# Tencent/hpc-ops

Measured on AMD Instinct MI355X. Metric: attention_decode_fp8_kv_throughput, higher is better.
Workload: dtype fp8_e4m3

## Files before the change

hpc-ops_amd/csrc/attention_decode_v2.hip:

```cpp
#include <atomic>
#include <type_traits>
#include <utility>

#include "hpc_common.h"
#include "hpc_dev.h"
#include "../../include/hpc_amd.h"
#include "attention_decode_v2.h"

namespace hpc {
namespace decode2 {

#ifdef HPC_DEV
__device__ int g_ticket_overruns;
#endif
constexpr int kThreads = 256;
constexpr int kWaves = 4;
constexpr float kNegInf = -__builtin_inff();
constexpr int kRow = 256;
constexpr int kRows = 32;
constexpr int kVOff = kRows * kRow;
constexpr int kWaveLds = 2 * kRows * kRow;

template <int kAux>
__device__ __forceinline__ void ld_x4x4(u32x4 (&k)[4], int voff, i32x4 rs_in, int s1, int s2, int s3) {
  const i32x4 rs = pin(rs_in);
  if constexpr (kAux == 2)
    asm volatile("s_nop 4\n\tbuffer_load_dwordx4 %0, %4, %5, 0 offen nt\n\tbuffer_load_dwordx4 %1, %4, %5, %6 offen nt\n\t"
                 "buffer_load_dwordx4 %2, %4, %5, %7 offen nt\n\tbuffer_load_dwordx4 %3, %4, %5, %8 offen nt"
                 : "=&v"(k[0]), "=&v"(k[1]), "=&v"(k[2]), "=&v"(k[3])
                 : "v"(voff), "s"(rs), "s"(s1), "s"(s2), "s"(s3));
  else
    asm volatile("s_nop 4\n\tbuffer_load_dwordx4 %0, %4, %5, 0 offen\n\tbuffer_load_dwordx4 %1, %4, %5, %6 offen\n\t"
                 "buffer_load_dwordx4 %2, %4, %5, %7 offen\n\tbuffer_load_dwordx4 %3, %4, %5, %8 offen"
                 : "=&v"(k[0]), "=&v"(k[1]), "=&v"(k[2]), "=&v"(k[3])
                 : "v"(voff), "s"(rs), "s"(s1), "s"(s2), "s"(s3));
}
__device__ __forceinline__ void ld_q3(u32x4 (&q)[2], uint32_t& sc, int voff_q, i32x4 rq_in, int voff_s, i32x4 rsc_in) {
  const i32x4 rq = pin(rq_in), rsc = pin(rsc_in);
  asm volatile("s_nop 4\n\tbuffer_load_dwordx4 %0, %3, %4, 0 offen\n\tbuffer_load_dwordx4 %1, %3, %4, 0 offen offset:64\n\t"
               "buffer_load_dword %2, %5, %6, 0 offen"
               : "=&v"(q[0]), "=&v"(q[1]), "=&v"(sc)
               : "v"(voff_q), "s"(rq), "v"(voff_s), "s"(rsc));
}
__device__ __forceinline__ void ld_q4(u32x4 (&q)[4], int voff_q, i32x4 rq_in) {
  const i32x4 rq = pin(rq_in);
  asm volatile("s_nop 4\n\tbuffer_load_dwordx4 %0, %4, %5, 0 offen\n\tbuffer_load_dwordx4 %1, %4, %5, 0 offen offset:64\n\t"
               "buffer_load_dwordx4 %2, %4, %5, 0 offen offset:128\n\tbuffer_load_dwordx4 %3, %4, %5, 0 offen offset:192"
               : "=&v"(q[0]), "=&v"(q[1]), "=&v"(q[2]), "=&v"(q[3])
               : "v"(voff_q), "s"(rq));
}
__device__ __forceinline__ void ld_ks(uint32_t& sc, int voff, i32x4 rs_in) {
  const i32x4 rs = pin(rs_in);
  asm volatile("s_nop 4\n\tbuffer_load_dword %0, %1, %2, 0 offen" : "=&v"(sc) : "v"(voff), "s"(rs));
}
template <int N>
__device__ __forceinline__ void wait_ks(uint32_t& sc) {
  asm volatile("s_waitcnt vmcnt(%1)" : "+v"(sc) : "n"(N));
}
template <int N>
__device__ __forceinline__ void wait_ks2(uint32_t& sc0, uint32_t& sc1) {
  asm volatile("s_waitcnt vmcnt(%2)" : "+v"(sc0), "+v"(sc1) : "n"(N));
}
template <int N>
__device__ __forceinline__ void wait_q8(u32x4 (&q0)[4], u32x4 (&q1)[4]) {
  asm volatile("s_waitcnt vmcnt(%8)"
               : "+v"(q0[0]), "+v"(q0[1]), "+v"(q0[2]), "+v"(q0[3]), "+v"(q1[0]), "+v"(q1[1]), "+v"(q1[2]), "+v"(q1[3])
               : "n"(N < 63 ? N : 63));
}
template <int N>
__device__ __forceinline__ void wait_x4x4(u32x4 (&k)[4]) {
  asm volatile("s_waitcnt vmcnt(%4)" : "+v"(k[0]), "+v"(k[1]), "+v"(k[2]), "+v"(k[3]) : "n"(N < 63 ? N : 63));
}
template <int N>
__device__ __forceinline__ void wait_q(u32x4 (&q0)[2], u32x4 (&q1)[2], uint32_t& s0, uint32_t& s1) {
  asm volatile("s_waitcnt vmcnt(%6)" : "+v"(q0[0]), "+v"(q0[1]), "+v"(q1[0]), "+v"(q1[1]), "+v"(s0), "+v"(s1) : "n"(N < 63 ? N : 63));
}


constexpr int kFValid = 1;
constexpr int kFLast = 2;
constexpr int kFFirst = 4;
constexpr int kFOn0 = 8;
constexpr int kFOn1 = 16;
constexpr int kFMasked = 32;

template <int kAux, bool kBf16 = false, bool kProf = false, bool kQuad = false, bool kKtok = false, bool kHnd = false, bool kSolo = false>
__global__ __launch_bounds__(kThreads, 2) void decode2_kernel(const Args a) {
  static_assert(!kSolo || (!kQuad && !kHnd), "one head per workgroup: fp8 (both quant types) or bf16");
  static_assert(!(kSolo && kBf16 && kKtok), "bf16 has no scales");
  static_assert(!(kBf16 && kQuad), "the quad form is fp8");
  static_assert(!kKtok || (!kBf16 && !kQuad), "per-token K scales: the fp8 head-pair form");
  static_assert(!kHnd || (!kBf16 && !kQuad && !kKtok), "HND pages: the fp8 head-pair form with per-tensor scales");
  __shared__ float s_ks[kKtok ? kWaves : 1][64];
  constexpr bool kWide = (kBf16 && !kSolo) || kQuad;
  constexpr bool kBSolo = kBf16 && kSolo;
  __shared__ __attribute__((aligned(1024))) uint8_t s_wave[kWaves][kWaveLds];
  __shared__ float s_m[2][kWaves][16];
  __shared__ float s_l[2][kWaves][16];
  __shared__ int s_ticket[2];
  constexpr int kH = kSolo ? 1 : kQuad ? 4 : 2;
  constexpr int kW = kBSolo ? 32 : kSolo ? 64 : kWide ? 16 : 32;
  constexpr int kRowB = kBSolo ? 256 : kSolo ? 128 : kWide ? 512 : 256;
  constexpr int kRpi = kBSolo ? 4 : (kHnd || kSolo) ? 8 : kWide ? 2 : 4;
  constexpr int kCpr = 64 / kRpi;

  const int tid = threadIdx.x;
  const int lane = tid & 63;
  const int wave = sgpr(tid >> 6);
  const int n = lane & 15;
  const int g = lane >> 4;
  const int wg = blockIdx.x, nwg = gridDim.x;
  const int B = a.num_batch, Sq = a.num_seq_q;
  const int G = 1 << a.g_shift;
  const int rows_valid = Sq << a.g_shift;
  auto row_ok = [&](int r16, int hh = 0) __attribute__((always_inline)) { return (kQuad ? (r16 & 7) : kSolo ? 16 * hh + r16 : r16) < rows_valid; };
  const int page_mask = (1 << a.page_shift) - 1;
  const cint_ptr lens = as_const(a.lens);
  const int mpl_tiles = as_const(a.task_map)[6] >> 6;
  const int add_new = a.new_kv_included ? 0 : Sq;
  const uint8_t* qbase = static_cast<const uint8_t*>(a.q);
  const auto part_rs = make_rsrc(a.part_o);
  const auto lse_rs = make_rsrc(a.part_lse);
  auto ltot_of = [&](int b) __attribute__((always_inline)) { const int l = lens[b] + add_new; return l > 0 ? l : 0; };
  auto tiles_of = [&](int b) __attribute__((always_inline)) { return (ltot_of(b) + 63) >> 6; };

  constexpr int kOvh = 2;
  auto cost_of = [&](int b) __attribute__((always_inline)) { const int t = tiles_of(b); return t > 0 ? t + kOvh : 0; };
  const int kpl = (B + 63) >> 6;
  int chunk_sum = 0;
  for (int i = 0; i < kpl; ++i) {
    const int b = lane * kpl + i;
    if (b < B) {
      const int l = a.lens[b] + add_new;
      const int t = ((l > 0 ? l : 0) + 63) >> 6;
      chunk_sum += t > 0 ? t + kOvh : 0;
    }
  }
  int incl = chunk_sum;
  incl += __builtin_amdgcn_update_dpp(0, incl, 0x111, 0xF, 0xF, false);
  incl += __builtin_amdgcn_update_dpp(0, incl, 0x112, 0xF, 0xF, false);
  incl += __builtin_amdgcn_update_dpp(0, incl, 0x114, 0xF, 0xF, false);
  incl += __builtin_amdgcn_update_dpp(0, incl, 0x118, 0xF, 0xF, false);
  incl += __builtin_amdgcn_update_dpp(0, incl, 0x142, 0xA, 0xF, false);
  incl += __builtin_amdgcn_update_dpp(0, incl, 0x143, 0xC, 0xF, false);
  const int chunk_start = incl - chunk_sum;
  const int Th = __builtin_amdgcn_readlane(incl, 63);
  const int npair = a.num_head_kv / kH;
  if (Th == 0) return;
  int nrange = nwg / npair;
  int rng = wg / npair;
  int pr = wg % npair;
  if (a.xcd_map != 0 && npair == 4 && (nwg & 7) == 0) {
    const int e = (a.xcd_map >> (3 * (wg & 7))) & 7;
    pr = e & 3;
    rng = (wg >> 3) * 2 + (e >> 2);
  }
  if (a.mate_from > 0 && wg >= a.mate_from) pr ^= a.pair_xor;
  if constexpr (kSolo) {
    if (a.share_shift > 0) {
      const int ss = a.share_shift, hk = npair >> ss;
      if (hk < 8 && (8 % hk) == 0 && (nrange % (8 / hk)) == 0) {
        const int x = wg & 7, j = wg >> 3;
        pr = ((x % hk) << ss) | (j & ((1 << ss) - 1));
        rng = (j >> ss) * (8 / hk) + x / hk;
      } else {
        pr = ((pr % hk) << ss) | (pr / hk);
      }
    }
  }
  int lwg = wg;
  int lwg0 = pr * nrange;
  if (a.pair_wgs[0] > 0 && npair == 4) {
    const int n0 = a.pair_wgs[0], n1 = a.pair_wgs[1], n2 = a.pair_wgs[2], n3 = a.pair_wgs[3];
    const int nmin = min(min(n0, n1), min(n2, n3));
    if (wg >= nmin * 4) {
      int e = wg - nmin * 4;
      pr = 0;
      rng = nmin + e;
      if (e >= n0 - nmin) { e -= n0 - nmin; pr = 1; rng = nmin + e;
        if (e >= n1 - nmin) { e -= n1 - nmin; pr = 2; rng = nmin + e;
          if (e >= n2 - nmin) { e -= n2 - nmin; pr = 3; rng = nmin + e; } } }
    }
    nrange = pr == 0 ? n0 : pr == 1 ? n1 : pr == 2 ? n2 : n3;
    lwg0 = pr == 0 ? 0 : pr == 1 ? n0 : pr == 2 ? n0 + n1 : n0 + n1 + n2;
  }
  lwg = lwg0 + rng;
  const int nbig = a.big_pct > 100 ? (nwg / 2) / npair : 0;
  const long denom = static_cast<long>(nbig) * a.big_pct + static_cast<long>(nrange - nbig) * 100;
  const int per_s_even = static_cast<int>((static_cast<long>(Th) * 100 + denom - 1) / denom);
  const int per_floor = a.min_range_cost > mpl_tiles ? a.min_range_cost : mpl_tiles;
  const int per_s = per_s_even > per_floor ? per_s_even : per_floor;
  const int per_b = nbig > 0 ? (per_s * a.big_pct + 99) / 100 : per_s;
  const int big_span = nbig * per_b;
  auto range_of = [&](int pos) __attribute__((always_inline)) { return pos < big_span ? pos / per_b : nbig + (pos - big_span) / per_s; };
  const long g_begin = rng < nbig ? static_cast<long>(rng) * per_b : big_span + static_cast<long>(rng - nbig) * per_s;
  const int per = rng < nbig ? per_b : per_s;
  const long g_end = g_begin + per < Th ? g_begin + per : Th;
  if (g_begin >= g_end) return;

  constexpr int kSnap = 16;
  const bool snap = per_s_even <= per_floor && !(kHpcDevBuild && a.dev_nosnap);
  auto locate = [&](int x, int& b_out, int& rt_out, int& cc_out) __attribute__((always_inline)) {
    if (x >= Th) {
      b_out = B;
      rt_out = 0;
      cc_out = Th;
      return;
    }
    const uint64_t le = __ballot(chunk_start <= x);
    const int cl = 63 - __builtin_clzll(le);
    int pos = __builtin_amdgcn_readlane(chunk_start, cl);
    int b = cl * kpl;
    while (true) {
      const int t = cost_of(b);
      if (x < pos + t) break;
      pos += t;
      ++b;
    }
    if (snap && x > pos) {
      const int t = cost_of(b);
      if (t - kOvh <= kSnap) {
        if (2 * (x - pos) >= t) {
          pos += t;
          ++b;
          while (b < B && cost_of(b) == 0) ++b;
          if (b >= B) {
            b_out = B;
            rt_out = 0;
            cc_out = Th;
            return;
          }
        }
        b_out = b;
        rt_out = 0;
        cc_out = pos;
        return;
      }
    }
    b_out = b;
    rt_out = x - pos > kOvh ? x - pos - kOvh : 0;
    cc_out = pos;
  };
  int c_b, c_rt0, c_cc, e_b, e_rt, e_cc;
  locate(static_cast<int>(g_begin), c_b, c_rt0, c_cc);
  locate(static_cast<int>(g_end), e_b, e_rt, e_cc);
  if (c_b == e_b && c_rt0 >= e_rt) return;

  int q0_b = 0, q0_ltot = 0, q0_end = 0, q0_cc = 0;
  int q1_b = 0, q1_ltot = 0, q1_end = 0, q1_cc = 0;
  int q2_b = 0, q2_ltot = 0, q2_end = 0, q2_cc = 0;
  int qn = 0;
  int c_tok = 0, c_tok_end = 0, c_ltot = 0, c_tiles = 0, c_first = 1, c_valid = 1, c_pending = 0, c_last = 0;
  cint_ptr c_row = as_const(a.block_ids);
  auto open_task = [&]() __attribute__((always_inline)) {
    c_ltot = ltot_of(c_b);
    c_tiles = (c_ltot + 63) >> 6;
    const int end_t = c_b == e_b ? e_rt : c_tiles;
    c_tok_end = end_t * 64 < c_ltot ? end_t * 64 : c_ltot;
    c_tok = c_rt0 * 64 + wave * kW;
    c_first = 1;
    c_row = as_const(a.block_ids) + static_cast<long>(c_b) * a.max_blocks;
    const bool e0 = qn == 0, e1 = qn == 1, e2 = qn >= 2;
    q0_b = e0 ? c_b : q0_b, q0_ltot = e0 ? c_ltot : q0_ltot, q0_end = e0 ? c_tok_end : q0_end, q0_cc = e0 ? c_cc : q0_cc;
    q1_b = e1 ? c_b : q1_b, q1_ltot = e1 ? c_ltot : q1_ltot, q1_end = e1 ? c_tok_end : q1_end, q1_cc = e1 ? c_cc : q1_cc;
    q2_b = e2 ? c_b : q2_b, q2_ltot = e2 ? c_ltot : q2_ltot, q2_end = e2 ? c_tok_end : q2_end, q2_cc = e2 ? c_cc : q2_cc;
    ++qn;
  };
  auto next_task = [&]() __attribute__((always_inline)) {
    if (c_b == e_b) {
      c_valid = 0;
      return;
    }
    c_cc += c_tiles + kOvh;
    do {
      ++c_b;
    } while (c_b < e_b && tiles_of(c_b) == 0);
    if (c_b == e_b && e_rt == 0) {
      c_valid = 0;
      return;
    }
    c_rt0 = 0;
    open_task();
  };
  const bool blk1_same_page = (1 << a.page_shift) >= kW;
  auto step = [&](int& tok, int& fl, int& pid0, int& pid1) __attribute__((always_inline)) {
    if (c_pending && c_valid) {
      if (c_last) {
        next_task();
      } else {
        c_tok += kWaves * kW;
        c_first = 0;
      }
    }
    c_pending = 1;
    c_last = c_tok + kWaves * kW >= c_tok_end;
    const bool on0 = c_valid && c_tok < c_tok_end, on1 = c_valid && c_tok + kW / 2 < c_tok_end;
    const bool masked = c_tok + kW > c_ltot - Sq + 1 || c_tok + kW > c_tok_end;
    fl = (c_valid ? kFValid : 0) | (c_last ? kFLast : 0) | (c_first ? kFFirst : 0) | (on0 ? kFOn0 : 0) | (on1 ? kFOn1 : 0) |
         (masked ? kFMasked : 0);
    tok = c_tok;
    pid0 = on0 ? c_row[c_tok >> a.page_shift] : 0;
    pid1 = (!blk1_same_page && on1) ? c_row[(c_tok + kW / 2) >> a.page_shift] : 0;
  };

  u32x4 kr[2][4];
  u32x4 vr[2][4];
  uint32_t qsc[2];
  const uint32_t k_rs = static_cast<uint32_t>(a.k_token_stride), v_rs = static_cast<uint32_t>(a.v_token_stride);
  const int in0 = (wave * kW) & page_mask;
  const int in1 = blk1_same_page ? in0 + kW / 2 : ((wave * kW + kW / 2) & page_mask);
  const int lane_off = (lane % kCpr) * 16;
  const int k_voff0 = static_cast<int>((in0 + lane / kCpr) * k_rs) + lane_off, k_voff1 = static_cast<int>((in1 + lane / kCpr) * k_rs) + lane_off;
  const int v_voff0 = static_cast<int>((in0 + lane / kCpr) * v_rs) + lane_off, v_voff1 = static_cast<int>((in1 + lane / kCpr) * v_rs) + lane_off;
  const int ks1 = sgpr(kRpi * k_rs), ks2 = sgpr(kHnd ? static_cast<uint32_t>(a.k_head_stride) : 2 * kRpi * k_rs);
  const int ks3 = sgpr(kHnd ? static_cast<uint32_t>(a.k_head_stride) + kRpi * k_rs : 3 * kRpi * k_rs);
  const int vs1 = sgpr(kRpi * v_rs), vs2 = sgpr(kHnd ? static_cast<uint32_t>(a.v_head_stride) : 2 * kRpi * v_rs);
  const int vs3 = sgpr(kHnd ? static_cast<uint32_t>(a.v_head_stride) + kRpi * v_rs : 3 * kRpi * v_rs);
  const int mem_slice = kSolo ? (pr >> a.share_shift) : (a.dev_slice > 0 ? a.dev_slice - 1 : pr);
  const uint64_t kbase_h = reinterpret_cast<uint64_t>(a.kcache) + static_cast<uint64_t>(mem_slice) * (kSolo ? static_cast<uint64_t>(a.k_head_stride) : kHnd ? 2 * static_cast<uint64_t>(a.k_head_stride) : kRowB);
  const uint64_t vbase_h = reinterpret_cast<uint64_t>(a.vcache) + static_cast<uint64_t>(mem_slice) * (kSolo ? static_cast<uint64_t>(a.v_head_stride) : kHnd ? 2 * static_cast<uint64_t>(a.v_head_stride) : kRowB);
  const uint32_t kbs = static_cast<uint32_t>(a.k_block_stride), vbs = static_cast<uint32_t>(a.v_block_stride);
  const bool mem = a.dev_nomem == 0;
  i32x4 dk0, dk1, dv0, dv1;
  uint32_t ksr = 0;
  uint32_t ksr1 = 0;
  i32x4 dks = i32x4{0, 0, 0, kSrdWord3};
  i32x4 dks1 = i32x4{0, 0, 0, kSrdWord3};
  const uint64_t ksbase_h = reinterpret_cast<uint64_t>(a.kscale) + static_cast<uint64_t>(mem_slice) * (kSolo ? 1 : 2) * a.ks_head_stride +
                            static_cast<uint64_t>(in0 >> 5) * a.ks_row_stride;
  const uint64_t ksbase1_h = reinterpret_cast<uint64_t>(a.kscale) + static_cast<uint64_t>(mem_slice) * a.ks_head_stride +
                             static_cast<uint64_t>(blk1_same_page ? (in0 >> 5) + 1 : in1 >> 5) * a.ks_row_stride;
  const uint32_t ksbs = static_cast<uint32_t>(a.ks_block_stride);
  auto make_descs = [&](int fl, int pid0, int pid1) __attribute__((always_inline)) {
    const int nrec0 = (fl & kFOn0) && mem ? -1 : 0, nrec1 = (fl & kFOn1) && mem ? -1 : 0;
    const uint64_t ka = kbase_h + static_cast<uint64_t>(static_cast<uint32_t>(pid0)) * kbs;
    const uint64_t va = vbase_h + static_cast<uint64_t>(static_cast<uint32_t>(pid0)) * vbs;
    dk0 = srd(static_cast<uint32_t>(ka), static_cast<uint32_t>(ka >> 32), nrec0);
    dv0 = srd(static_cast<uint32_t>(va), static_cast<uint32_t>(va >> 32), nrec0);
    if (blk1_same_page) {
      dk1 = i32x4{dk0[0], dk0[1], sgpr(nrec1), kSrdWord3};
      dv1 = i32x4{dv0[0], dv0[1], sgpr(nrec1), kSrdWord3};
    } else {
      const uint64_t kb = kbase_h + static_cast<uint64_t>(static_cast<uint32_t>(pid1)) * kbs;
      const uint64_t vb = vbase_h + static_cast<uint64_t>(static_cast<uint32_t>(pid1)) * vbs;
      dk1 = srd(static_cast<uint32_t>(kb), static_cast<uint32_t>(kb >> 32), nrec1);
      dv1 = srd(static_cast<uint32_t>(vb), static_cast<uint32_t>(vb >> 32), nrec1);
    }
    if constexpr (kKtok) {
      const uint64_t sa = ksbase_h + static_cast<uint64_t>(static_cast<uint32_t>(pid0)) * ksbs;
      dks = srd(static_cast<uint32_t>(sa), static_cast<uint32_t>(sa >> 32), (fl & kFOn0) ? (kSolo ? 128 : 256) : 0);
      if constexpr (kSolo) {
        const uint64_t sb = ksbase1_h + static_cast<uint64_t>(static_cast<uint32_t>(blk1_same_page ? pid0 : pid1)) * ksbs;
        dks1 = srd(static_cast<uint32_t>(sb), static_cast<uint32_t>(sb >> 32), (fl & kFOn1) ? 128 : 0);
      }
    }
  };
  auto issue_k0 = [&]() __attribute__((always_inline)) { ld_x4x4<kAux>(kr[0], k_voff0, dk0, ks1, ks2, ks3); };
  auto issue_k1 = [&]() __attribute__((always_inline)) { ld_x4x4<kAux>(kr[1], k_voff1, dk1, ks1, ks2, ks3); };
  auto issue_v0 = [&]() __attribute__((always_inline)) { ld_x4x4<kAux>(vr[0], v_voff0, dv0, vs1, vs2, vs3); };
  auto issue_v1 = [&]() __attribute__((always_inline)) { ld_x4x4<kAux>(vr[1], v_voff1, dv1, vs1, vs2, vs3); };
  auto issue_ks = [&]() __attribute__((always_inline)) {
    if constexpr (kKtok && kSolo) {
      ld_ks(ksr, (lane & 31) * 4, dks);
      ld_ks(ksr1, (lane & 31) * 4, dks1);
    } else if constexpr (kKtok) {
      ld_ks(ksr, lane * 4, dks);
    }
  };

  uint8_t* my_lds = s_wave[wave];
  float* my_so = reinterpret_cast<float*>(my_lds);
  const uint32_t lds0 = static_cast<uint32_t>(reinterpret_cast<uintptr_t>((lds_u8*)my_lds));
  const int tj = (lane & 15) >> 1;
  const int ttok = 16 * (tj >> 2) + 4 * g + (tj & 3);
  const int btok = 4 * g + ((lane & 15) >> 2);
  const int bkey = ((btok << 1) & 15) | (btok >> 3);
  const int qtok = 4 * (g & 1) + (tj & 3) + 8 * (tj >> 2);
  const uint32_t w0_inv = (kSolo && !kBf16) ? lds0 + (lane >> 3) * kRowB + (((lane & 7) ^ (lane >> 3)) * 16)
                          : kHnd ? lds0 + (lane >> 3) * kRowB + (((lane & 7) ^ (lane >> 3)) * 16)
                          : kWide ? lds0 + (lane >> 5) * kRowB + (((lane & 31) ^ (lane >> 5)) * 16)
                                  : lds0 + (lane >> 4) * kRowB + (((lane & 15) ^ (lane >> 4)) * 16);
  const uint32_t w1_inv = kBSolo ? lds0 + kVOff + (lane >> 4) * kRowB + (((lane & 15) ^ ((lane >> 4) << 1)) * 16)
                                 : lds0 + kVOff + (lane >> 5) * kRowB + (((lane & 31) ^ ((lane >> 5) << 1)) * 16);
  const uint32_t r0_inv = (kSolo && !kBf16) ? lds0 + n * kRowB + ((g ^ (n & 7)) * 16) : lds0 + n * kRowB + ((g ^ n) * 16);
  const uint32_t t0_inv = kBSolo ? lds0 + kVOff + btok * kRowB + (((((lane & 3) >> 1) ^ ((btok & 3) << 1))) * 16) + (lane & 1) * 8
                          : kBf16 ? lds0 + kVOff + btok * kRowB + (((((lane & 3) >> 1) ^ bkey)) * 16) + (lane & 1) * 8
                          : kSolo ? lds0 + kVOff + ttok * kRowB + ((((ttok & 7) ^ (((ttok >> 4) & 1) << 2))) * 16) + (lane & 1) * 8
                          : kQuad ? lds0 + kVOff + qtok * kRowB + ((((g >> 1) << 3) ^ qtok) * 16) + (lane & 1) * 8
                                  : lds0 + kVOff + ttok * kRowB + ((((ttok & 15) ^ ((ttok >> 4) << 3))) * 16) + (lane & 1) * 8;
  const uint32_t p_keep = (n >> 3) == (g >> 1) ? 0xffffffffu : 0u;

  u32x4 qf[2][kBf16 ? 4 : 2];
  float row_scale[2];
  float out_scale;
  float out_scale_h[2] = {0.f, 0.f};
  f32x4 o[2][8];
  float m_run[2], l_run[2];
  auto load_q = [&](int db) __attribute__((always_inline)) {
    if constexpr (kBSolo) {
      const i32x4 rq = srd_of(qbase + static_cast<long>(db) * Sq * a.ldq + (pr << a.g_shift) * 256,
                              static_cast<unsigned>((Sq - 1) * a.ldq + G * 256));
#pragma unroll
      for (int hh = 0; hh < 2; ++hh) {
        const int r = 16 * hh + n;
        ld_q4(qf[hh], (r >> a.g_shift) * a.ldq + (r & (G - 1)) * 256 + g * 16, rq);
      }
      return;
    }
    if constexpr (kBf16) {
      const int q_voff = (n >> a.g_shift) * a.ldq + (n & (G - 1)) * 256 + g * 16;
      const i32x4 rq = srd_of(qbase + static_cast<long>(db) * Sq * a.ldq + ((pr * kH) << a.g_shift) * 256,
                              static_cast<unsigned>((Sq - 1) * a.ldq + kH * G * 256));
      ld_q4(qf[0], q_voff, rq);
      ld_q4(qf[1], q_voff + G * 256, rq);
      return;
    }
    if constexpr (kQuad) {
      const int r8 = n & 7, hl = n >> 3;
      const bool okc = r8 < rows_valid;
      const int q_voff = okc ? (r8 >> a.g_shift) * a.ldq + ((hl << a.g_shift) + (r8 & (G - 1))) * 128 + g * 16 : -256;
      const int s_voff = okc ? ((r8 >> a.g_shift) * a.qscale_stride + (hl << a.g_shift) + (r8 & (G - 1))) * 4 : -256;
      const i32x4 rq = srd_of(qbase + static_cast<long>(db) * Sq * a.ldq + ((pr * kH) << a.g_shift) * 128,
                              static_cast<unsigned>((Sq - 1) * a.ldq + kH * G * 128));
      const i32x4 rsq = srd_of(a.qscale + static_cast<long>(db) * Sq * a.qscale_stride + ((pr * kH) << a.g_shift),
                               static_cast<unsigned>(((Sq - 1) * a.qscale_stride + kH * G) * 4));
      ld_q3(reinterpret_cast<u32x4(&)[2]>(qf[0]), qsc[0], q_voff, rq, s_voff, rsq);
      ld_q3(reinterpret_cast<u32x4(&)[2]>(qf[1]), qsc[1], okc ? q_voff + 2 * G * 128 : -256, rq, okc ? s_voff + 2 * G * 4 : -256, rsq);
      return;
    }
    if constexpr (kSolo) {
      const i32x4 rq = srd_of(qbase + static_cast<long>(db) * Sq * a.ldq + (pr << a.g_shift) * 128,
                              static_cast<unsigned>((Sq - 1) * a.ldq + G * 128));
      const i32x4 rsq = srd_of(a.qscale + static_cast<long>(db) * Sq * a.qscale_stride + (pr << a.g_shift),
                               static_cast<unsigned>(((Sq - 1) * a.qscale_stride + G) * 4));
#pragma unroll
      for (int hh = 0; hh < 2; ++hh) {
        const int r = 16 * hh + n;
        ld_q3(reinterpret_cast<u32x4(&)[2]>(qf[hh]), qsc[hh], (r >> a.g_shift) * a.ldq + (r & (G - 1)) * 128 + g * 16, rq,
              ((r >> a.g_shift) * a.qscale_stride + (r & (G - 1))) * 4, rsq);
      }
      return;
    }
    const int q_voff = (n >> a.g_shift) * a.ldq + (n & (G - 1)) * 128 + g * 16;
    const int s_voff = ((n >> a.g_shift) * a.qscale_stride + (n & (G - 1))) * 4;
    const i32x4 rq = srd_of(qbase + static_cast<long>(db) * Sq * a.ldq + ((pr * kH) << a.g_shift) * 128,
                            static_cast<unsigned>((Sq - 1) * a.ldq + kH * G * 128));
    const i32x4 rsq = srd_of(a.qscale + static_cast<long>(db) * Sq * a.qscale_stride + ((pr * kH) << a.g_shift),
                             static_cast<unsigned>(((Sq - 1) * a.qscale_stride + kH * G) * 4));
    if constexpr (!kBf16) {
      ld_q3(reinterpret_cast<u32x4(&)[2]>(qf[0]), qsc[0], q_voff, rq, s_voff, rsq);
      ld_q3(reinterpret_cast<u32x4(&)[2]>(qf[1]), qsc[1], q_voff + G * 128, rq, s_voff + G * 4, rsq);
    }
  };
  auto reset_state = [&]() __attribute__((always_inline)) {
#pragma unroll
    for (int hh = 0; hh < 2; ++hh)
#pragma unroll
      for (int jj = 0; jj < 8; ++jj) o[hh][jj] = f32x4{0.f, 0.f, 0.f, 0.f};
#pragma unroll
    for (int hh = 0; hh < 2; ++hh) {
      m_run[hh] = kNegInf;
      l_run[hh] = 0.f;
    }
  };

  int p1_tok, p1_fl, p2_tok, p2_fl, p2_pid0, p2_pid1;

  auto combine4 = [&](int hh, int row16, int c8, float (&acc)[8], float& M, float& L) __attribute__((always_inline)) {
    float mw[kWaves];
    M = kNegInf;
#pragma unroll
    for (int w = 0; w < kWaves; ++w) {
      mw[w] = s_m[hh][w][row16];
      M = fmaxf(M, mw[w]);
    }
    const float Mu = M == kNegInf ? 0.f : M;
    L = 0.f;
#pragma unroll
    for (int i = 0; i < 8; ++i) acc[i] = 0.f;
#pragma unroll
    for (int w = 0; w < kWaves; ++w) {
      const float wgt = __builtin_amdgcn_exp2f(mw[w] - Mu);
      L += wgt * s_l[hh][w][row16];
      const float* so = reinterpret_cast<const float*>(s_wave[w]) + (hh * 16 + row16) * 128 + c8 * 8;
      const f32x4 x0 = *reinterpret_cast<const f32x4*>(so);
      const f32x4 x1 = *reinterpret_cast<const f32x4*>(so + 4);
#pragma unroll
      for (int i = 0; i < 4; ++i) {
        acc[i] = fmaf(wgt, x0[i], acc[i]);
        acc[4 + i] = fmaf(wgt, x1[i], acc[4 + i]);
      }
    }
  };
  auto store_y = [&](int db, int hh, int row16, int c8, const float (&acc)[8], float inv) __attribute__((always_inline)) {
    const int qrow = kQuad ? (row16 & 7) : kSolo ? 16 * hh + row16 : row16;
    const int rs = qrow >> a.g_shift;
    const int h = kQuad ? pr * kH + hh * 2 + (row16 >> 3) : kSolo ? pr : pr * kH + hh;
    uint16_t* dst = a.y + (static_cast<long>(db) * Sq + rs) * a.ldy + ((h << a.g_shift) + (qrow & (G - 1))) * 128 + c8 * 8;
    u32x4 pk;
#pragma unroll
    for (int i = 0; i < 4; ++i) pk[i] = pack_bf16x2(acc[2 * i] * inv, acc[2 * i + 1] * inv);
    st16(dst, pk);
  };

  int np = 0, p0_b = 0, p0_first = 0, p0_n = 0, p1_b = 0, p1_first = 0, p1_n = 0;
  auto merge_request = [&](int db, int first_rng, int nchunks) __attribute__((always_inline)) {
    int* cnt = a.arrive + static_cast<long>(pr) * B + db;
    const int r4 = lane >> 4, c8l = lane & 15;
    auto slot_of = [&](int c, int hh) __attribute__((always_inline)) {
      return (static_cast<long>(lwg0 + first_rng + c) * 2 + (c == 0 ? 1 : 0)) * 2 + hh;
    };
#pragma unroll 1
    for (int ig = 0; ig < 2; ++ig) {
      if (!kQuad && ig * 8 >= rows_valid) break;
      float um[2][2], ul[2][2], ua[2][2][8];
#pragma unroll
      for (int hh = 0; hh < 2; ++hh)
#pragma unroll
        for (int i = 0; i < 2; ++i) {
          um[hh][i] = kNegInf;
          ul[hh][i] = 0.f;
#pragma unroll
          for (int e = 0; e < 8; ++e) ua[hh][i][e] = 0.f;
        }
      for (int c0 = wave; c0 < nchunks; c0 += 2 * kWaves) {
        float lv[2][2][2];
        u32x4 x0[2][2][2], x1[2][2][2];
#pragma unroll
        for (int u = 0; u < 2; ++u) {
          const int c = c0 + u * kWaves < nchunks ? c0 + u * kWaves : c0;
          if (u > 0 && c0 + u * kWaves >= nchunks && !(kHpcDevBuild && a.dev_merge_dup)) continue;
#pragma unroll
          for (int hh = 0; hh < 2; ++hh) {
            const long slot = slot_of(c, hh);
#pragma unroll
            for (int i = 0; i < 2; ++i) {
              const int row = ig * 8 + i * 4 + r4;
              lv[u][hh][i] = __uint_as_float(__builtin_amdgcn_raw_buffer_load_b32(lse_rs, static_cast<int>((slot * 16 + row) * 4), 0, 16));
              const int off = static_cast<int>(((slot * 16 + row) * 128 + c8l * 8) * 4);
              x0[u][hh][i] = __builtin_amdgcn_raw_buffer_load_b128(part_rs, off, 0, 16);
              x1[u][hh][i] = __builtin_amdgcn_raw_buffer_load_b128(part_rs, off + 16, 0, 16);
            }
          }
        }
#pragma unroll
        for (int u = 0; u < 2; ++u) {
          const bool real = c0 + u * kWaves < nchunks;
          if (!real && !(kHpcDevBuild && a.dev_merge_dup)) continue;
#pragma unroll
          for (int hh = 0; hh < 2; ++hh)
#pragma unroll
            for (int i = 0; i < 2; ++i) {
              const float lse = real ? lv[u][hh][i] : kNegInf;
              const float mn = fmaxf(um[hh][i], lse);
              const float mu = mn == kNegInf ? 0.f : mn;
              const float sc_old = __builtin_amdgcn_exp2f(um[hh][i] - mu), wgt = __builtin_amdgcn_exp2f(lse - mu);
              um[hh][i] = mn;
              ul[hh][i] = ul[hh][i] * sc_old + wgt;
#pragma unroll
              for (int e = 0; e < 4; ++e) {
                ua[hh][i][e] = fmaf(wgt, __uint_as_float(x0[u][hh][i][e]), ua[hh][i][e] * sc_old);
                ua[hh][i][4 + e] = fmaf(wgt, __uint_as_float(x1[u][hh][i][e]), ua[hh][i][4 + e] * sc_old);
              }
            }
        }
      }
#pragma unroll
      for (int hh = 0; hh < 2; ++hh)
#pragma unroll
        for (int i = 0; i < 2; ++i) {
          const int row = ig * 8 + i * 4 + r4;
          if (c8l == 0) {
            s_m[hh][wave][row] = um[hh][i];
            s_l[hh][wave][row] = ul[hh][i];
          }
          float* so = my_so + (hh * 16 + row) * 128 + c8l * 8;
          *reinterpret_cast<f32x4*>(so) = f32x4{ua[hh][i][0], ua[hh][i][1], ua[hh][i][2], ua[hh][i][3]};
          *reinterpret_cast<f32x4*>(so + 4) = f32x4{ua[hh][i][4], ua[hh][i][5], ua[hh][i][6], ua[hh][i][7]};
        }
    }
    __syncthreads();
    const int row16 = tid >> 4, c8 = tid & 15;
#pragma unroll
    for (int hh = 0; hh < 2; ++hh) {
      if (row_ok(row16, hh)) {
        float acc[8], M, L;
        combine4(hh, row16, c8, acc, M, L);
        store_y(db, hh, row16, c8, acc, L > 0.f ? 1.0f / L : 0.f);
      }
    }
    if (tid == 0) __hip_atomic_store(cnt, 0, __ATOMIC_RELAXED, __HIP_MEMORY_SCOPE_AGENT);
    __syncthreads();
  };
  auto flush_pending = [&]() __attribute__((always_inline)) {
    if (np == 0) return;
    asm volatile("s_waitcnt vmcnt(0)" ::: "memory");
    __syncthreads();
    if (tid == 0) {
      s_ticket[0] = __hip_atomic_fetch_add(a.arrive + static_cast<long>(pr) * B + p0_b, 1, __ATOMIC_RELAXED, __HIP_MEMORY_SCOPE_AGENT) + 1;
      if (np > 1)
        s_ticket[1] = __hip_atomic_fetch_add(a.arrive + static_cast<long>(pr) * B + p1_b, 1, __ATOMIC_RELAXED, __HIP_MEMORY_SCOPE_AGENT) + 1;
    }
    __syncthreads();
    const int t0 = s_ticket[0], t1 = s_ticket[1];
#ifdef HPC_DEV
    if (tid == 0 && (t0 > p0_n || (np > 1 && t1 > p1_n))) atomicAdd(&g_ticket_overruns, 1);
#endif
    if (t0 == p0_n) merge_request(p0_b, p0_first, p0_n);
    if (np > 1 && t1 == p1_n) merge_request(p1_b, p1_first, p1_n);
    np = 0;
  };

  auto finish_task = [&]() __attribute__((always_inline)) {
    const int db = q0_b;
    const int d_tiles = (q0_ltot + 63) >> 6;
    const bool whole = snap && d_tiles <= kSnap;
    const int first_rng = whole ? rng : range_of(q0_cc + kOvh);
    const int nchunks = whole ? 1 : range_of(q0_cc + kOvh + d_tiles - 1) - first_rng + 1;
    const int ichunk = rng - first_rng;
#pragma unroll
    for (int hh = 0; hh < 2; ++hh) {
      const float l = row4_sum(l_run[hh]);
      if (g == 0) {
        s_m[hh][wave][n] = m_run[hh];
        s_l[hh][wave][n] = l;
      }
#pragma unroll
      for (int jj = 0; jj < 8; ++jj)
        *reinterpret_cast<f32x4*>(&my_so[(hh * 16 + n) * 128 + jj * 16 + g * 4]) = o[hh][jj];
    }
    __syncthreads();
    {
      const int row16 = tid >> 4, c8 = tid & 15;
#pragma unroll
      for (int hh = 0; hh < 2; ++hh) {
        float acc[8], M, L;
        combine4(hh, row16, c8, acc, M, L);
        const float inv = (L > 0.f ? 1.0f / L : 0.f) * (kKtok ? out_scale_h[hh] : out_scale);
        if (row_ok(row16, hh)) {
          if (nchunks == 1) {
            store_y(db, hh, row16, c8, acc, inv);
          } else {
            const long slot = (static_cast<long>(lwg) * 2 + (ichunk == 0 ? 1 : 0)) * 2 + hh;
            const int off = static_cast<int>(((slot * 16 + row16) * 128 + c8 * 8) * 4);
            __builtin_amdgcn_raw_buffer_store_b128(u32x4{__float_as_uint(acc[0] * inv), __float_as_uint(acc[1] * inv), __float_as_uint(acc[2] * inv),
                                                         __float_as_uint(acc[3] * inv)}, part_rs, off, 0, 16);
            __builtin_amdgcn_raw_buffer_store_b128(u32x4{__float_as_uint(acc[4] * inv), __float_as_uint(acc[5] * inv), __float_as_uint(acc[6] * inv),
                                                         __float_as_uint(acc[7] * inv)}, part_rs, off + 16, 0, 16);
            if (c8 == 0)
              __builtin_amdgcn_raw_buffer_store_b32(__float_as_uint(L > 0.f ? M + __builtin_amdgcn_logf(L) - (kBf16 ? 0.0f : 8.0f) : kNegInf),
                                                    lse_rs, static_cast<int>((slot * 16 + row16) * 4), 0, 16);
          }
        }
      }
    }
    if (nchunks > 1) {
      p1_b = np == 1 ? db : p1_b, p1_first = np == 1 ? first_rng : p1_first, p1_n = np == 1 ? nchunks : p1_n;
      p0_b = np == 0 ? db : p0_b, p0_first = np == 0 ? first_rng : p0_first, p0_n = np == 0 ? nchunks : p0_n;
      np = np < 2 ? np + 1 : 2;
    }
    __syncthreads();
    reset_state();
    q0_b = q1_b, q0_ltot = q1_ltot, q0_end = q1_end, q0_cc = q1_cc;
    q1_b = q2_b, q1_ltot = q2_ltot, q1_end = q2_end, q1_cc = q2_cc;
    --qn;
    if (p1_fl & kFValid) load_q(q0_b);
  };

  reset_state();
#pragma unroll
  for (int hh = 0; hh < 2; ++hh) {
#pragma unroll
    for (int c = 0; c < (kBf16 ? 4 : 2); ++c) qf[hh][c] = u32x4{0u, 0u, 0u, 0u};
    qsc[hh] = 0u;
  }
#pragma unroll
  for (int hh = 0; hh < 2; ++hh) row_scale[hh] = 0.f;
  out_scale = 0.f;
  open_task();
  step(p2_tok, p2_fl, p2_pid0, p2_pid1);
  make_descs(p2_fl, sgpr(p2_pid0), sgpr(p2_pid1));
  issue_k0();
  issue_k1();
  issue_ks();
  issue_v0();
  issue_v1();
  p1_tok = p2_tok;
  p1_fl = p2_fl;
  load_q(q0_b);
  step(p2_tok, p2_fl, p2_pid0, p2_pid1);

  uint64_t pf_wk = 0, pf_wr = 0, pf_wv = 0, pf_is = 0, pf_cp = 0, pf_fin = 0, pf_n = 0, pf_t0 = 0, pf_r0 = 0, pf_last = 0;
  auto now = [&]() __attribute__((always_inline)) -> uint64_t { return kProf ? __builtin_amdgcn_s_memtime() : 0; };
  if constexpr (kProf) {
    pf_t0 = now();
    pf_r0 = __builtin_amdgcn_s_memrealtime();
  }
  while (true) {
    const int d_tok = p1_tok, d_fl = p1_fl;
    if (!(d_fl & kFValid)) break;
    pf_last = now();
    uint32_t w0 = w0_inv, w1 = w1_inv, r0 = r0_inv, t0 = t0_inv;
    asm volatile("" : "+v"(w0), "+v"(w1), "+v"(r0), "+v"(t0));
    make_descs(p2_fl, sgpr(p2_pid0), sgpr(p2_pid1));
    p1_tok = p2_tok;
    p1_fl = p2_fl;
    auto write_k = [&](int tb) __attribute__((always_inline)) {
#pragma unroll
      for (int q = 0; q < 4; ++q) {
        if constexpr (kSolo && !kBf16)
          *reinterpret_cast<lds_u32x4*>(static_cast<uint32_t>((w0 ^ (((q >> 1) << 2) * 16)) + (tb * 32 + q * 8) * kRowB)) = kr[tb][q];
        else if constexpr (kHnd)
          *reinterpret_cast<lds_u32x4*>(static_cast<uint32_t>((w0 ^ ((((q >> 1) << 3) ^ ((q & 1) << 3) ^ (tb << 3)) * 16)) + (tb * 16 + (q & 1) * 8) * kRowB)) = kr[tb][q];
        else if constexpr (kWide)
          *reinterpret_cast<lds_u32x4*>(static_cast<uint32_t>((w0 ^ (((q << 1) ^ (tb << 3)) * 16)) + (tb * 8 + q * 2) * kRowB)) = kr[tb][q];
        else
          *reinterpret_cast<lds_u32x4*>(static_cast<uint32_t>((w0 ^ (((q << 2) ^ (tb << 3)) * 16)) + (tb * 16 + q * 4) * kRowB)) = kr[tb][q];
      }
    };
    auto write_v = [&](int tb) __attribute__((always_inline)) {
#pragma unroll
      for (int q = 0; q < 4; ++q) {
        if constexpr (kBSolo)
          *reinterpret_cast<lds_u32x4*>(static_cast<uint32_t>(w1 + (tb * 16 + q * 4) * kRowB)) = vr[tb][q];
        else if constexpr (kSolo)
          *reinterpret_cast<lds_u32x4*>(static_cast<uint32_t>((w0 ^ (((q >> 1) << 2) * 16)) + kVOff + (tb * 32 + q * 8) * kRowB)) = vr[tb][q];
        else if constexpr (kHnd)
          *reinterpret_cast<lds_u32x4*>(static_cast<uint32_t>((w0 ^ ((((q >> 1) << 3) ^ ((q & 1) << 3) ^ (tb << 3)) * 16)) + kVOff + (tb * 16 + (q & 1) * 8) * kRowB)) = vr[tb][q];
        else if constexpr (kBf16)
          *reinterpret_cast<lds_u32x4*>(static_cast<uint32_t>((w1 ^ (((q << 2) ^ tb) * 16)) + (tb * 8 + q * 2) * kRowB)) = vr[tb][q];
        else if constexpr (kQuad)
          *reinterpret_cast<lds_u32x4*>(static_cast<uint32_t>((w0 ^ (((q << 1) ^ (tb << 3)) * 16)) + kVOff + (tb * 8 + q * 2) * kRowB)) = vr[tb][q];
        else
          *reinterpret_cast<lds_u32x4*>(static_cast<uint32_t>((w0 ^ (((q << 2) ^ (tb << 3)) * 16)) + kVOff + (tb * 16 + q * 4) * kRowB)) = vr[tb][q];
      }
    };
    auto q_ready = [&]() __attribute__((always_inline)) {
      if (d_fl & kFFirst) {
        if constexpr (kBf16) {
          wait_q8<0>(qf[0], qf[1]);
          row_scale[0] = row_scale[1] = a.scale_log2;
          out_scale = 1.0f;
        } else {
          wait_q<0>(reinterpret_cast<u32x4(&)[2]>(qf[0]), reinterpret_cast<u32x4(&)[2]>(qf[1]), qsc[0], qsc[1]);
          const float kmul = kKtok ? 1.0f : as_constf(a.kscale)[0];
#pragma unroll
          for (int hh = 0; hh < 2; ++hh) row_scale[hh] = a.scale_log2 * __uint_as_float(qsc[hh]) * kmul;
          out_scale = as_constf(a.vscale)[0];
          if constexpr (kKtok) {
            out_scale_h[0] = as_constf(a.vscale)[kSolo ? (pr >> a.share_shift) : pr * 2];
            out_scale_h[1] = as_constf(a.vscale)[kSolo ? (pr >> a.share_shift) : pr * 2 + 1];
          }
        }
      }
    };
    constexpr int kNks = kKtok ? (kSolo ? 2 : 1) : 0;
    wait_x4x4<12 + kNks>(kr[0]);
    wait_x4x4<8 + kNks>(kr[1]);
    if constexpr (kProf) { const uint64_t t = now(); pf_wk += t - pf_last; pf_last = t; }
    write_k(0);
    write_k(1);
    if constexpr (kKtok && kSolo) {
      wait_ks2<8>(ksr, ksr1);
      s_ks[wave][lane] = __uint_as_float(lane < 32 ? ksr : ksr1);
    } else if constexpr (kKtok) {
      wait_ks<8>(ksr);
      s_ks[wave][lane] = __uint_as_float(ksr);
    }
    if constexpr (kProf) { const uint64_t t = now(); pf_wr += t - pf_last; pf_last = t; }
    wait_x4x4<4>(vr[0]);
    wait_x4x4<0>(vr[1]);
    if constexpr (kProf) { const uint64_t t = now(); pf_wv += t - pf_last; pf_last = t; }
    write_v(0);
    write_v(1);
    if constexpr (kProf) { const uint64_t t = now(); pf_wr += t - pf_last; pf_last = t; }
    if constexpr (kHpcDevBuild) {
      if (a.dev_sleep > 0 && !(pr & 1))
        for (int i = 0; i < a.dev_sleep; ++i) __builtin_amdgcn_s_sleep(1);
    }
    issue_k0();
    issue_k1();
    issue_ks();
    issue_v0();
    issue_v1();
    q_ready();
    step(p2_tok, p2_fl, p2_pid0, p2_pid1);
    if constexpr (kProf) { const uint64_t t = now(); pf_is += t - pf_last; pf_last = t; }

    if constexpr (kBSolo) {
      f32x4 sacc[2][2];
#pragma unroll
      for (int tb = 0; tb < 2; ++tb) {
        f32x4 acc[2] = {f32x4{0.f, 0.f, 0.f, 0.f}, f32x4{0.f, 0.f, 0.f, 0.f}};
#pragma unroll
        for (int j = 0; j < 4; ++j) {
          const u32x4 kk = *reinterpret_cast<const lds_u32x4*>(static_cast<uint32_t>((r0 ^ (((j << 2) ^ (tb << 3)) * 16)) + tb * 16 * kRowB));
#pragma unroll
          for (int hh = 0; hh < 2; ++hh)
            acc[hh] = __builtin_amdgcn_mfma_f32_16x16x32_bf16(__builtin_bit_cast(bf16x8, kk), __builtin_bit_cast(bf16x8, qf[hh][j]), acc[hh], 0, 0, 0);
        }
        sacc[0][tb] = acc[0];
        sacc[1][tb] = acc[1];
      }
      v4i16 pf[2][2];
#pragma unroll
      for (int hh = 0; hh < 2; ++hh)
#pragma unroll
        for (int tb = 0; tb < 2; ++tb)
#pragma unroll
          for (int r = 0; r < 4; ++r) sacc[hh][tb][r] *= row_scale[hh];
      if (d_fl & kFMasked) {
#pragma unroll
        for (int hh = 0; hh < 2; ++hh) {
          const int sq_row = (16 * hh + n) >> a.g_shift;
          const int lim = (q0_end - 1 < q0_ltot - Sq + sq_row) ? q0_end - 1 : q0_ltot - Sq + sq_row;
#pragma unroll
          for (int tb = 0; tb < 2; ++tb)
#pragma unroll
            for (int r = 0; r < 4; ++r) sacc[hh][tb][r] = (d_tok + tb * 16 + g * 4 + r) <= lim ? sacc[hh][tb][r] : kNegInf;
        }
      }
#pragma unroll
      for (int hh = 0; hh < 2; ++hh) {
        float mt = kNegInf;
#pragma unroll
        for (int tb = 0; tb < 2; ++tb)
#pragma unroll
          for (int r = 0; r < 4; ++r) mt = __builtin_fmaxf(mt, sacc[hh][tb][r]);
        mt = row4_max(mt);
        const float m_new = fmaxf(m_run[hh], mt);
        const float m_use = m_new == kNegInf ? 0.f : m_new;
        float psum = 0.f;
#pragma unroll
        for (int tb = 0; tb < 2; ++tb) {
          float prb[4];
#pragma unroll
          for (int r = 0; r < 4; ++r) {
            prb[r] = __builtin_amdgcn_exp2f(sacc[hh][tb][r] - m_use);
            psum += prb[r];
          }
          pf[hh][tb] = __builtin_bit_cast(v4i16, u32x2{pack_bf16x2(prb[0], prb[1]), pack_bf16x2(prb[2], prb[3])});
        }
        if (__builtin_amdgcn_ballot_w64(m_new != m_run[hh]) != 0) {
          const float alpha = __builtin_amdgcn_exp2f(m_run[hh] - m_use);
          l_run[hh] *= alpha;
#pragma unroll
          for (int jj = 0; jj < 8; ++jj) o[hh][jj] *= alpha;
          m_run[hh] = m_new;
        }
        l_run[hh] += psum;
      }
#pragma unroll
      for (int tb = 0; tb < 2; ++tb) {
        v4i16 vt[8];
#pragma unroll
        for (int u = 0; u < 8; ++u)
          vt[u] = __builtin_amdgcn_ds_read_tr16_b64_v4i16(
              reinterpret_cast<lds_v4i16*>(static_cast<uint32_t>((t0 ^ ((u << 1) * 16)) + tb * 16 * kRowB)));
        __builtin_amdgcn_sched_barrier(0);
#pragma unroll
        for (int hh = 0; hh < 2; ++hh)
#pragma unroll
          for (int u = 0; u < 8; ++u)
            o[hh][u] = __builtin_amdgcn_mfma_f32_16x16x16bf16_1k(vt[u], pf[hh][tb], o[hh][u], 0, 0, 0);
        __builtin_amdgcn_sched_barrier(0);
      }
    } else if constexpr (kBf16) {
      f32x4 sacc[2];
#pragma unroll
      for (int hh = 0; hh < 2; ++hh) {
        f32x4 acc = f32x4{0.f, 0.f, 0.f, 0.f};
#pragma unroll
        for (int j = 0; j < 4; ++j) {
          const u32x4 kk = *reinterpret_cast<const lds_u32x4*>(static_cast<uint32_t>(r0 ^ (((hh << 4) ^ (j << 2)) * 16)));
          acc = __builtin_amdgcn_mfma_f32_16x16x32_bf16(__builtin_bit_cast(bf16x8, kk), __builtin_bit_cast(bf16x8, qf[hh][j]), acc, 0, 0, 0);
        }
        sacc[hh] = acc;
      }
      v4i16 pf[2];
#pragma unroll
      for (int hh = 0; hh < 2; ++hh) {
#pragma unroll
        for (int r = 0; r < 4; ++r) sacc[hh][r] *= row_scale[hh];
      }
      if (d_fl & kFMasked) {
        const int sq_row = n >> a.g_shift;
        const int lim = (q0_end - 1 < q0_ltot - Sq + sq_row) ? q0_end - 1 : q0_ltot - Sq + sq_row;
#pragma unroll
        for (int hh = 0; hh < 2; ++hh)
#pragma unroll
          for (int r = 0; r < 4; ++r) sacc[hh][r] = (d_tok + g * 4 + r) <= lim ? sacc[hh][r] : kNegInf;
      }
#pragma unroll
      for (int hh = 0; hh < 2; ++hh) {
        float mt = __builtin_fmaxf(__builtin_fmaxf(sacc[hh][0], sacc[hh][1]), __builtin_fmaxf(sacc[hh][2], sacc[hh][3]));
        mt = row4_max(mt);
        const float m_new = fmaxf(m_run[hh], mt);
        const float m_use = m_new == kNegInf ? 0.f : m_new;
        float prb[4], psum = 0.f;
#pragma unroll
        for (int r = 0; r < 4; ++r) {
          prb[r] = __builtin_amdgcn_exp2f(sacc[hh][r] - m_use);
          psum += prb[r];
        }
        const uint32_t p01 = pack_bf16x2(prb[0], prb[1]), p23 = pack_bf16x2(prb[2], prb[3]);
        pf[hh] = __builtin_bit_cast(v4i16, u32x2{p01, p23});
        if (__builtin_amdgcn_ballot_w64(m_new != m_run[hh]) != 0) {
          const float alpha = __builtin_amdgcn_exp2f(m_run[hh] - m_use);
          l_run[hh] *= alpha;
#pragma unroll
          for (int jj = 0; jj < 8; ++jj) o[hh][jj] *= alpha;
          m_run[hh] = m_new;
        }
        l_run[hh] += psum;
      }
#pragma unroll
      for (int hh = 0; hh < 2; ++hh) {
        v4i16 vt[8];
#pragma unroll
        for (int u = 0; u < 8; ++u)
          vt[u] = __builtin_amdgcn_ds_read_tr16_b64_v4i16(
              reinterpret_cast<lds_v4i16*>(static_cast<uint32_t>(t0 ^ (((hh << 4) ^ (u << 1)) * 16))));
        __builtin_amdgcn_sched_barrier(0);
#pragma unroll
// ... 364 lines not shown
```

Measured before the change: 5728.

## Prefetch next task's Q before combine barrier and relax vmcnt waits

Moves the load of the next task's Q to before the combine __syncthreads so it overlaps the cross-wave reduction. The vmcnt waits on the K/V tiles are adjusted to account for the in-flight Q loads on first tiles, and the Q wait is relaxed so it need not drain all outstanding loads. K and V scale constants are hoisted out of the per-task path and read once at kernel start. For small batches, per-batch lengths are fetched through readlane from a lane-held value instead of global reads. The counter arithmetic is subtle, and a wrong count could let data be read before it arrives.

```diff
diff --git a/hpc-ops_amd/csrc/attention_decode_v2.hip b/hpc-ops_amd/csrc/attention_decode_v2.hip
--- a/hpc-ops_amd/csrc/attention_decode_v2.hip
+++ b/hpc-ops_amd/csrc/attention_decode_v2.hip
@@ -76,6 +76,11 @@
   asm volatile("s_waitcnt vmcnt(%6)" : "+v"(q0[0]), "+v"(q0[1]), "+v"(q1[0]), "+v"(q1[1]), "+v"(s0), "+v"(s1) : "n"(N < 63 ? N : 63));
 }
 
+
+template <int N>
+__device__ __forceinline__ void wait_plain() {
+  asm volatile("s_waitcnt vmcnt(%0)" ::"n"(N));
+}
 
 constexpr int kFValid = 1;
 constexpr int kFLast = 2;
@@ -121,18 +126,25 @@
   const uint8_t* qbase = static_cast<const uint8_t*>(a.q);
   const auto part_rs = make_rsrc(a.part_o);
   const auto lse_rs = make_rsrc(a.part_lse);
-  auto ltot_of = [&](int b) __attribute__((always_inline)) { const int l = lens[b] + add_new; return l > 0 ? l : 0; };
+  const int kpl = (B + 63) >> 6;
+  int lane_ltot = 0;
+  auto ltot_of = [&](int b) __attribute__((always_inline)) {
+    if (kpl == 1) return __builtin_amdgcn_readlane(lane_ltot, b);
+    const int l = lens[b] + add_new;
+    return l > 0 ? l : 0;
+  };
   auto tiles_of = [&](int b) __attribute__((always_inline)) { return (ltot_of(b) + 63) >> 6; };
 
   constexpr int kOvh = 2;
   auto cost_of = [&](int b) __attribute__((always_inline)) { const int t = tiles_of(b); return t > 0 ? t + kOvh : 0; };
-  const int kpl = (B + 63) >> 6;
   int chunk_sum = 0;
   for (int i = 0; i < kpl; ++i) {
     const int b = lane * kpl + i;
     if (b < B) {
       const int l = a.lens[b] + add_new;
-      const int t = ((l > 0 ? l : 0) + 63) >> 6;
+      const int lc = l > 0 ? l : 0;
+      if (i == 0) lane_ltot = lc;
+      const int t = (lc + 63) >> 6;
       chunk_sum += t > 0 ? t + kOvh : 0;
     }
   }
@@ -392,8 +404,7 @@
 
   u32x4 qf[2][kBf16 ? 4 : 2];
   float row_scale[2];
-  float out_scale;
-  float out_scale_h[2] = {0.f, 0.f};
+  float k_mul = 1.0f, v_mul = 1.0f, v_mul_h[2] = {1.0f, 1.0f};
   f32x4 o[2][8];
   float m_run[2], l_run[2];
   auto load_q = [&](int db) __attribute__((always_inline)) {
@@ -629,6 +640,7 @@
       for (int jj = 0; jj < 8; ++jj)
         *reinterpret_cast<f32x4*>(&my_so[(hh * 16 + n) * 128 + jj * 16 + g * 4]) = o[hh][jj];
     }
+    if (p1_fl & kFValid) load_q(q1_b);
     __syncthreads();
     {
       const int row16 = tid >> 4, c8 = tid & 15;
@@ -636,7 +648,7 @@
       for (int hh = 0; hh < 2; ++hh) {
         float acc[8], M, L;
         combine4(hh, row16, c8, acc, M, L);
-        const float inv = (L > 0.f ? 1.0f / L : 0.f) * (kKtok ? out_scale_h[hh] : out_scale);
+        const float inv = (L > 0.f ? 1.0f / L : 0.f) * (kKtok ? v_mul_h[hh] : v_mul);
         if (row_ok(row16, hh)) {
           if (nchunks == 1) {
             store_y(db, hh, row16, c8, acc, inv);
@@ -664,7 +676,6 @@
     q0_b = q1_b, q0_ltot = q1_ltot, q0_end = q1_end, q0_cc = q1_cc;
     q1_b = q2_b, q1_ltot = q2_ltot, q1_end = q2_end, q1_cc = q2_cc;
     --qn;
-    if (p1_fl & kFValid) load_q(q0_b);
   };
 
   reset_state();
@@ -676,7 +687,6 @@
   }
 #pragma unroll
   for (int hh = 0; hh < 2; ++hh) row_scale[hh] = 0.f;
-  out_scale = 0.f;
   open_task();
   step(p2_tok, p2_fl, p2_pid0, p2_pid1);
   make_descs(p2_fl, sgpr(p2_pid0), sgpr(p2_pid1));
@@ -689,6 +699,13 @@
   p1_fl = p2_fl;
   load_q(q0_b);
   step(p2_tok, p2_fl, p2_pid0, p2_pid1);
+  if constexpr (kKtok) {
+    v_mul_h[0] = as_constf(a.vscale)[kSolo ? (pr >> a.share_shift) : pr * 2];
+    v_mul_h[1] = as_constf(a.vscale)[kSolo ? (pr >> a.share_shift) : pr * 2 + 1];
+  } else if constexpr (!kBf16) {
+    k_mul = as_constf(a.kscale)[0];
+    v_mul = as_constf(a.vscale)[0];
+  }
 
   uint64_t pf_wk = 0, pf_wr = 0, pf_wv = 0, pf_is = 0, pf_cp = 0, pf_fin = 0, pf_n = 0, pf_t0 = 0, pf_r0 = 0, pf_last = 0;
   auto now = [&]() __attribute__((always_inline)) -> uint64_t { return kProf ? __builtin_amdgcn_s_memtime() : 0; };
@@ -735,41 +752,40 @@
           *reinterpret_cast<lds_u32x4*>(static_cast<uint32_t>((w0 ^ (((q << 2) ^ (tb << 3)) * 16)) + kVOff + (tb * 16 + q * 4) * kRowB)) = vr[tb][q];
       }
     };
+    constexpr int kNks = kKtok ? (kSolo ? 2 : 1) : 0;
+    constexpr int kNq = kBf16 ? 8 : 6;
+    const bool first = (d_fl & kFFirst) != 0;
     auto q_ready = [&]() __attribute__((always_inline)) {
-      if (d_fl & kFFirst) {
+      if (first) {
         if constexpr (kBf16) {
-          wait_q8<0>(qf[0], qf[1]);
+          wait_q8<16 + kNks>(qf[0], qf[1]);
           row_scale[0] = row_scale[1] = a.scale_log2;
-          out_scale = 1.0f;
         } else {
-          wait_q<0>(reinterpret_cast<u32x4(&)[2]>(qf[0]), reinterpret_cast<u32x4(&)[2]>(qf[1]), qsc[0], qsc[1]);
-          const float kmul = kKtok ? 1.0f : as_constf(a.kscale)[0];
-#pragma unroll
-          for (int hh = 0; hh < 2; ++hh) row_scale[hh] = a.scale_log2 * __uint_as_float(qsc[hh]) * kmul;
-          out_scale = as_constf(a.vscale)[0];
-          if constexpr (kKtok) {
-            out_scale_h[0] = as_constf(a.vscale)[kSolo ? (pr >> a.share_shift) : pr * 2];
-            out_scale_h[1] = as_constf(a.vscale)[kSolo ? (pr >> a.share_shift) : pr * 2 + 1];
-          }
+          wait_q<16 + kNks>(reinterpret_cast<u32x4(&)[2]>(qf[0]), reinterpret_cast<u32x4(&)[2]>(qf[1]), qsc[0], qsc[1]);
+#pragma unroll
+          for (int hh = 0; hh < 2; ++hh) row_scale[hh] = a.scale_log2 * __uint_as_float(qsc[hh]) * k_mul;
         }
       }
     };
-    constexpr int kNks = kKtok ? (kSolo ? 2 : 1) : 0;
-    wait_x4x4<12 + kNks>(kr[0]);
-    wait_x4x4<8 + kNks>(kr[1]);
+    if (!first) wait_plain<8 + kNks>();
+    wait_x4x4<12 + kNks + kNq>(kr[0]);
+    wait_x4x4<8 + kNks + kNq>(kr[1]);
     if constexpr (kProf) { const uint64_t t = now(); pf_wk += t - pf_last; pf_last = t; }
     write_k(0);
     write_k(1);
     if constexpr (kKtok && kSolo) {
-      wait_ks2<8>(ksr, ksr1);
+      if (!first) wait_plain<8>();
+      wait_ks2<8 + kNq>(ksr, ksr1);
       s_ks[wave][lane] = __uint_as_float(lane < 32 ? ksr : ksr1);
     } else if constexpr (kKtok) {
-      wait_ks<8>(ksr);
+      if (!first) wait_plain<8>();
+      wait_ks<8 + kNq>(ksr);
       s_ks[wave][lane] = __uint_as_float(ksr);
     }
     if constexpr (kProf) { const uint64_t t = now(); pf_wr += t - pf_last; pf_last = t; }
-    wait_x4x4<4>(vr[0]);
-    wait_x4x4<0>(vr[1]);
+    if (!first) wait_plain<0>();
+    wait_x4x4<4 + kNq>(vr[0]);
+    wait_x4x4<kNq>(vr[1]);
     if constexpr (kProf) { const uint64_t t = now(); pf_wv += t - pf_last; pf_last = t; }
     write_v(0);
     write_v(1);
```

Result: no change. 5775, median of 5 (+0.8%).
